# xinntao/EDVR

Measured on AMD Instinct MI355X. Metric: EDVR-L x4 5-frame 720p clips/sec, higher is better.
Workload: dtype fp32 emulated as 2xf16 (hi+lo, 22-bit operands, 4 cross products), fp32 accumulate; 1 GPU; EDVR-L x4, 5 frames, 180x320 LR -> 720x1280, batch 10/GPU, inference; clips_per_gpu=10, global_clips=10, parallelism=clip-sharded x1, no data-path collective, world_size=1, backend=single process

## Files before the change

### edvr_amd/_lib.py

```python
import ctypes
import os

_HERE = os.path.dirname(os.path.abspath(__file__))
LIB_PATH = os.environ.get('EDVR_AMD_LIB') or os.path.join(_HERE, 'lib', 'libedvr_amd.so')

c_float_p = ctypes.c_void_p
i32, i64, f32, sz = ctypes.c_int, ctypes.c_int64, ctypes.c_float, ctypes.c_size_t
vp = ctypes.c_void_p


class ConvDesc(ctypes.Structure):
    _fields_ = [
        ('x1', vp), ('x2', vp), ('c1', i32), ('c2', i32), ('x1_img_stride', i64), ('x2_img_stride', i64),
        ('x2_div', i32), ('x2_mul', i32), ('x2_add', i32), ('n', i32), ('h', i32), ('w', i32), ('wpk', vp),
        ('bias', vp), ('co', i32), ('ks', i32), ('stride', i32), ('act', i32), ('act_from', i32), ('res1', vp),
        ('res2', vp), ('res1_img_stride', i64), ('res2_img_stride', i64), ('y', vp), ('y_img_stride', i64),
        ('out_mode', i32), ('algo', i32), ('gate', vp), ('gate_img_stride', i64), ('gate_slope', f32), ('y_scale', f32),
        ('wpk_f4', vp), ('abs_sum', vp), ('abs_sum_channels', i32), ('wpk_f4s', vp), ('x_amax', vp), ('y_amax', vp),
        ('pre', vp), ('pre_img_stride', i64), ('pre_div', i32), ('pre_mul', i32), ('pre_add', i32), ('pre_n', i32),
    ]


PROTOTYPES = {
    'edvr_version': (ctypes.c_char_p, []),
# ... 9 lines not shown
    'edvr_conv2d_pack_weight_1x1s_f32': (i32, [vp, vp, i32, i32, vp]),
    'edvr_amax_f32': (i32, [vp, vp, i32, i64, i64, vp]),
    'edvr_pack_job_bytes': (sz, []),
    'edvr_conv2d_pack_weights_multi': (i32, [vp, i32, i32, i32, vp]),
    'edvr_conv2d_f32': (i32, [ctypes.POINTER(ConvDesc), vp]),
    'edvr_conv2d_gate_supported': (i32, [ctypes.POINTER(ConvDesc)]),
    'edvr_conv2d_abs_sum_supported': (i32, [ctypes.POINTER(ConvDesc)]),
    'edvr_conv2d_y_amax_supported': (i32, [ctypes.POINTER(ConvDesc)]),
    'edvr_conv2d_pre_supported': (i32, [ctypes.POINTER(ConvDesc)]),
    'edvr_conv2d_kernel_name': (i32, [ctypes.POINTER(ConvDesc), ctypes.c_char_p, sz]),
    'edvr_conv2d_executed_flops': (i32, [ctypes.POINTER(ConvDesc), ctypes.POINTER(ctypes.c_double)]),
    'edvr_dcnv2_fwd_ws_bytes': (sz, [i32] * 12),
    'edvr_dcnv2_fwd_f32': (i32, [vp] * 6 + [i32] * 12 + [i64, i64, i32, i32, vp, sz, vp]),
    'edvr_dcnv2_fwd_split_f32': (i32, [vp] * 6 + [i32] * 12 + [i64, i64, i32, i32, vp, sz, vp, vp]),
    'edvr_dcnv2_fwd_split_applies': (i32, [vp] + [i32] * 13),
    'edvr_dcnv2_fwd_kernel_name': (i32, [vp] + [i32] * 13 + [ctypes.c_char_p, sz]),
    'edvr_dcnv2_bwd_ws_bytes': (sz, [i32] * 12),
    'edvr_dcnv2_any_ws_bytes': (sz, [i32] * 13),
    'edvr_dcnv2_fwd_any': (i32, [i32] + [vp] * 6 + [i32] * 12 + [i64, i64, vp, sz, vp]),
    'edvr_dcnv2_bwd_any': (i32, [i32] + [vp] * 10 + [i32] * 12 + [i64, i64, i64, i64, vp, sz, vp]),
    'edvr_psnr_sse_f32': (i32, [vp, vp, vp, i32, i32, i32, i32, i64, i64, i32, i32, i32, vp]),
    'edvr_ssim_partials': (sz, [i32, i32, i32]),
    'edvr_ssim_f32': (i32, [vp, vp, vp, i32, i32, i32, i32, i64, i64, i32, i32, vp]),
    'edvr_frames_u8_to_f32': (i32, [vp, vp, i32, i32, i32, i32, vp, i32, vp]),
    'edvr_gather_images_f32': (i32, [vp, vp, vp, vp, i32, vp, i32, i32, vp]),
    'edvr_upsample4x_add_u8': (i32, [vp, vp, vp, i32, i32, i32, vp]),
    'edvr_f32_to_u8_hwc': (i32, [vp, vp, i32, i32, i32, i64, vp]),
    'edvr_crop_pad_frames_u8': (i32, [vp, vp, i32, i32, i32, i32, i32, i32, i32, i32, vp]),
    'edvr_crop_pad_frames_f32': (i32, [vp, vp, i32, i32, i32, i64, i32, i32, i32, i32, i32, vp]),
    'edvr_upsample4x_add_rect_f32': (i32, [vp, vp, vp, i32, i32, i32, i32, i32, i32, i32, i64, i64, i64, vp]),
# ... 89 lines not shown
```

### edvr_amd/csrc/common.h

```cpp
#pragma once
#include <hip/hip_runtime.h>

#include <cstdarg>
#include <cstdio>

#include "../../include/edvr_amd.h"

namespace edvr {

void set_error(const char *fmt, ...);

inline int check_launch(const char *what) {
  hipError_t e = hipGetLastError();
  if (e != hipSuccess) {
    set_error("%s: %s", what, hipGetErrorString(e));
    return EDVR_ERR_LAUNCH;
  }
  return EDVR_OK;
}

inline hipStream_t as_stream(edvr_stream_t s) { return reinterpret_cast<hipStream_t>(s); }

inline int cdiv(int a, int b) { return (a + b - 1) / b; }
inline int64_t cdiv64(int64_t a, int64_t b) { return (a + b - 1) / b; }
// ... 66 lines not shown
  int64_t doff_bs, dmsk_bs;
};
int dcn_fill_shape(DcnShape &s, int B, int C, int H, int W, int Co, int kh, int kw, int stride, int pad, int dil, int groups, int dg,
                   int64_t off_bs, int64_t msk_bs);

bool dcn_fused_supported(int C, int Co, int H, int W, int kh, int kw, int stride, int pad, int dil, int groups, int dg);
int dcn_fused_pack(const float *weight, float *wpk, int Co, int C, hipStream_t stream);
int dcn_fused_forward(const float *x, const float *offset, const float *mask, const float *wpk, const float *bias, float *y, int B, int C,
                      int H, int W, int Co, int dg, int64_t off_bs, int64_t msk_bs, int act, int halo, hipStream_t stream);

bool dcn_tapwin_supported(int C, int Co, int H, int W, int kh, int kw, int stride, int pad, int dil, int groups, int dg);
int dcn_tapwin_forward(const float *x, const float *offset, const float *mask, const float *wpk, const float *bias, float *y, int B, int C,
                       int H, int W, int Co, int dg, int64_t off_bs, int64_t msk_bs, int act, hipStream_t stream);

bool dcn_tapwin_split_enabled();
int dcn_tapwin_split_forward(const float *x, const float *offset, const float *mask, const float *weight, unsigned *wpk, const float *bias, float *y,
                             int B, int C, int H, int W, int Co, int dg, int64_t off_bs, int64_t msk_bs, int act, const float *xm_amax,
                             hipStream_t stream);

bool dcn_bwd_fused_supported(const DcnShape &s);
size_t dcn_bwd_fused_wbk_elems(int dg);
int dcn_bwd_fused_launch(const DcnShape &s, const float *x, const float *offset, const float *mask, const float *weight, const float *dy,
                         float *wbk, float *col, float *dx, float *doffset, float *dmask, hipStream_t stream);

__device__ inline int xcd_remap(int linear, int total) {
  const int q = total >> 3, rem = total & 7, xcd = linear & 7;
  return xcd * q + (xcd < rem ? xcd : rem) + (linear >> 3);
}
__device__ inline void xcd_block_index(int &bx, int &by, int &bz) {
  const int gx = gridDim.x, gy = gridDim.y;
  const int lin = blockIdx.x + gx * (blockIdx.y + gy * blockIdx.z);
// ... 16 lines not shown
```

### edvr_amd/csrc/dcn.hip

```cpp
#include <cstdlib>

#include "common.h"
#include "dcn_tap.h"

namespace edvr {

typedef float f32x16 __attribute__((ext_vector_type(16)));

__global__ void fill_kernel(float *__restrict__ p, float v, int64_t n) {
  for (int64_t i = (int64_t)blockIdx.x * blockDim.x + threadIdx.x; i < n; i += (int64_t)gridDim.x * blockDim.x) p[i] = v;
}

struct Merge {
  bool give01, give11;
  bool take00, take10;
};
__device__ __forceinline__ Merge merge_right(const Tap &t, bool same_plane_as_next) {
  Merge mg;
  const int lane = __lane_id();
  const int n_o00 = lane_next_i(t.o00), n_o10 = lane_next_i(t.o10);
  const int n_ok = lane_next_i((t.ok00 ? 1 : 0) | (t.ok10 ? 2 : 0));
  const bool has_next = lane < 63 && same_plane_as_next;
  mg.give01 = has_next && t.ok01 && (n_ok & 1) && n_o00 == t.o01;
  mg.give11 = has_next && t.ok11 && (n_ok & 2) && n_o10 == t.o11;
// ... 567 lines not shown
  edvr::DcnShape s;
  if (edvr::dcn_fill_shape(s, B, C, H, W, Co, kh, kw, stride, pad, dil, groups, dg, 0, 0)) return 0;
  return edvr::fwd_ws(s).total;
}

size_t edvr_dcnv2_bwd_ws_bytes(int B, int C, int H, int W, int Co, int kh, int kw, int stride, int pad, int dil, int groups,
                               int dg) {
  edvr::DcnShape s;
  if (edvr::dcn_fill_shape(s, B, C, H, W, Co, kh, kw, stride, pad, dil, groups, dg, 0, 0)) return 0;
  return edvr::bwd_ws(s).total;
}

static int dcnv2_fwd_impl(const float *x, const float *offset, const float *mask, const float *weight, const float *bias,
                          float *y, int B, int C, int H, int W, int Co, int kh, int kw, int stride, int pad, int dil, int groups,
                          int dg, int64_t offset_bstride, int64_t mask_bstride, int act, int halo_hint, void *ws, size_t ws_bytes,
                          const float *xm_amax, edvr_stream_t stream_) {
  using namespace edvr;
  EDVR_REQUIRE(x && offset && mask && weight && y, "dcnv2_fwd: null pointer");
  DcnShape s;
  int rc = dcn_fill_shape(s, B, C, H, W, Co, kh, kw, stride, pad, dil, groups, dg, offset_bstride, mask_bstride);
  if (rc) return rc;
  const FwdWs wsz = fwd_ws(s);
  if (!ws || ws_bytes < wsz.total) {
    set_error("dcnv2_fwd: workspace %zu < required %zu", ws_bytes, wsz.total);
    return EDVR_ERR_WORKSPACE;
  }
  hipStream_t stream = as_stream(stream_);
  const int K = kh * kw;
  const int64_t P = (int64_t)s.Ho * s.Wo;
  float *col = reinterpret_cast<float *>(static_cast<char *>(ws) + wsz.col);
  float *wpk = reinterpret_cast<float *>(static_cast<char *>(ws) + wsz.wpk);
  if (use_fused(s) && halo_hint == EDVR_DCN_HALO_TAPWIN && xm_amax && dcn_tapwin_split_enabled() &&
      dcn_tapwin_supported(C, Co, H, W, kh, kw, s.stride, s.pad, s.dil, groups, dg) && (reinterpret_cast<uintptr_t>(x) & 15) == 0)
    return dcn_tapwin_split_forward(x, offset, mask, weight, reinterpret_cast<unsigned *>(wpk), bias, y, B, C, H, W, Co, dg, s.off_bs, s.msk_bs, act,
                                    xm_amax, stream);
  if (use_fused(s) && halo_hint >= 0) {
    rc = dcn_fused_pack(weight, wpk, Co, C, stream);
    if (rc) return rc;
    if (halo_hint == EDVR_DCN_HALO_TAPWIN) {
      if (dcn_tapwin_supported(C, Co, H, W, kh, kw, s.stride, s.pad, s.dil, groups, dg) && (reinterpret_cast<uintptr_t>(x) & 15) == 0)
        return dcn_tapwin_forward(x, offset, mask, wpk, bias, y, B, C, H, W, Co, dg, s.off_bs, s.msk_bs, act, stream);
      halo_hint = 7;
    }
    return dcn_fused_forward(x, offset, mask, wpk, bias, y, B, C, H, W, Co, dg, s.off_bs, s.msk_bs, act, halo_hint, stream);
  }
  const int cig = C / groups, cog = Co / groups;
  const size_t wpk_g = edvr_conv2d_packed_weight_elems(cog, cig * K, 1);
  for (int g = 0; g < groups; ++g) {
    rc = edvr_conv2d_pack_weight_f32(weight + (size_t)g * cog * cig * K, wpk + g * wpk_g, cog, cig * K, 1, 0, stream_);
    if (rc) return rc;
// ... 15 lines not shown
    d.act = act;
    d.y = y + (int64_t)g * cog * P;
    d.y_img_stride = (int64_t)Co * P;
    d.out_mode = EDVR_OUT_NCHW;
    rc = conv2d_launch(d, stream);
    if (rc) return rc;
  }
  return EDVR_OK;
}

int edvr_dcnv2_fwd_f32(const float *x, const float *offset, const float *mask, const float *weight, const float *bias,
                       float *y, int B, int C, int H, int W, int Co, int kh, int kw, int stride, int pad, int dil, int groups,
                       int dg, int64_t offset_bstride, int64_t mask_bstride, int act, int halo_hint, void *ws, size_t ws_bytes,
                       edvr_stream_t stream) {
  return dcnv2_fwd_impl(x, offset, mask, weight, bias, y, B, C, H, W, Co, kh, kw, stride, pad, dil, groups, dg, offset_bstride, mask_bstride, act,
                        halo_hint, ws, ws_bytes, nullptr, stream);
}

int edvr_dcnv2_fwd_split_f32(const float *x, const float *offset, const float *mask, const float *weight, const float *bias,
                             float *y, int B, int C, int H, int W, int Co, int kh, int kw, int stride, int pad, int dil, int groups,
                             int dg, int64_t offset_bstride, int64_t mask_bstride, int act, int halo_hint, void *ws, size_t ws_bytes,
                             const float *xm_amax, edvr_stream_t stream) {
  EDVR_REQUIRE(xm_amax != nullptr, "dcnv2_fwd_split: null magnitude bound");
  return dcnv2_fwd_impl(x, offset, mask, weight, bias, y, B, C, H, W, Co, kh, kw, stride, pad, dil, groups, dg, offset_bstride, mask_bstride, act,
                        halo_hint, ws, ws_bytes, xm_amax, stream);
}

int edvr_dcnv2_fwd_split_applies(const float *x, int B, int C, int H, int W, int Co, int kh, int kw, int stride, int pad, int dil, int groups,
                                 int dg, int halo_hint) {
  using namespace edvr;
  DcnShape s;
  if (dcn_fill_shape(s, B, C, H, W, Co, kh, kw, stride, pad, dil, groups, dg, 0, 0)) return 0;
  return (use_fused(s) && halo_hint == EDVR_DCN_HALO_TAPWIN && dcn_tapwin_split_enabled() &&
          dcn_tapwin_supported(C, Co, H, W, kh, kw, s.stride, s.pad, s.dil, groups, dg) && (reinterpret_cast<uintptr_t>(x) & 15) == 0) ? 1 : 0;
}

int edvr_dcnv2_fwd_kernel_name(const float *x, int B, int C, int H, int W, int Co, int kh, int kw, int stride, int pad, int dil, int groups,
                               int dg, int halo_hint, char *buf, size_t buf_len) {
  using namespace edvr;
  EDVR_REQUIRE(buf && buf_len > 0, "dcnv2_fwd_kernel_name: null buffer");
  DcnShape s;
// ... 189 lines not shown
```

### edvr_amd/csrc/dcn_tapwin_s.hip

```cpp
#include <type_traits>

#include "common.h"
#include <cstdlib>

#include "dcn_tap.h"
#include "pack.h"

namespace edvr {

typedef float f32x16 __attribute__((ext_vector_type(16)));
typedef float f32x4 __attribute__((ext_vector_type(4)));
typedef float f32x2 __attribute__((ext_vector_type(2)));

namespace {
constexpr int TWS_TH = 8, TWS_TW = 32, TWS_RY = 2, TWS_RX = 2;
constexpr int TWS_IH = TWS_TH + 2 * TWS_RY;
constexpr int TWS_IW = (TWS_TW + 2 * TWS_RX + 3 + 3) / 4 * 4;
constexpr int TWS_PPR = TWS_IW / 4;
constexpr int TWS_HR = TWS_IH / 2;
constexpr int TWS_HB = TWS_HR * TWS_IW;
constexpr int TWS_CHS = TWS_IH * TWS_IW;
static_assert(TWS_HR * TWS_PPR <= 64 && TWS_IH == 2 * TWS_HR && TWS_CHS % 64 == 32, "window halves must fit one wave instruction");
constexpr int TWS_MAX_DG = 8;
constexpr int TWS_OOB = (int)0x80000000;
// ... 34 lines not shown

static __device__ __forceinline__ __amdgpu_buffer_rsrc_t tws_rsrc(const void *ptr, int bytes) {
  const uint64_t pv = reinterpret_cast<uint64_t>(ptr);
  const uint64_t pu = ((uint64_t)(uint32_t)__builtin_amdgcn_readfirstlane((int)(pv >> 32)) << 32) |
                      (uint32_t)__builtin_amdgcn_readfirstlane((int)(uint32_t)pv);
  return __builtin_amdgcn_make_buffer_rsrc(reinterpret_cast<void *>(pu), (short)0, bytes, TWS_RSRC_FLAGS);
}

static __device__ __forceinline__ void tws_split4(const float (&x)[4], unsigned (&o)[4]) {
  asm volatile(
      "v_fma_mixlo_f16 %0, %4, 1.0, 0\n\tv_fma_mixlo_f16 %1, %5, 1.0, 0\n\tv_fma_mixlo_f16 %2, %6, 1.0, 0\n\tv_fma_mixlo_f16 %3, %7, 1.0, 0\n\t"
      "v_fma_mixhi_f16 %0, %4, 1.0, -%0 op_sel_hi:[0,0,1]\n\tv_fma_mixhi_f16 %1, %5, 1.0, -%1 op_sel_hi:[0,0,1]\n\t"
      "v_fma_mixhi_f16 %2, %6, 1.0, -%2 op_sel_hi:[0,0,1]\n\tv_fma_mixhi_f16 %3, %7, 1.0, -%3 op_sel_hi:[0,0,1]"
      : "=&v"(o[0]), "=&v"(o[1]), "=&v"(o[2]), "=&v"(o[3])
      : "v"(x[0]), "v"(x[1]), "v"(x[2]), "v"(x[3]));
}

template <int MT, int CPG>
__global__ __launch_bounds__(256, 2) void dcn_tapwin_split_fwd_kernel(const DcnTapwinSArgs a) {
  constexpr int TH = TWS_TH, TW = TWS_TW, IH = TWS_IH, IW = TWS_IW, CHS = TWS_CHS, KK = 9, OOB = TWS_OOB;
  constexpr int MB = 32 * MT, NQ = CPG / 2, KG = CPG / 8;
  constexpr int XW = CPG * CHS;
  constexpr int WS = CPG * MB;
  constexpr int CPW = CPG / 4;
  static_assert(CPG % 4 == 0, "four waves share the channels of a group");
  __shared__ __attribute__((aligned(16))) float xw[2 * XW];
  __shared__ __attribute__((aligned(16))) unsigned wsl[2 * WS];
  __shared__ int shifts[TWS_MAX_DG * 18];
  __shared__ float tpl[4 * 3 * 64];

// ... 82 lines not shown
  };
  auto origin = [&](int g, int t, int &wy0, int &wx0) {
    const int sy = __builtin_amdgcn_readfirstlane(shifts[(g * KK + t) * 2]);
    const int sx = __builtin_amdgcn_readfirstlane(shifts[(g * KK + t) * 2 + 1]);
    const int ti = t / 3, tj = t - 3 * ti;
    wy0 = ty0 - 1 + ti + sy - TWS_RY;
    wx0 = (tx0 - 1 + tj + sx - TWS_RX) & ~3;
  };
  const i32x4 off_rsrc4 = tws_rsrc4(off_b, a.dg * 18 * P * 4), msk_rsrc4 = tws_rsrc4(msk_b, a.dg * 9 * P * 4);
  const unsigned tpl_lds = (unsigned)(size_t)(lvoid *)tpl + wave * (3 * 64 * 4);
  const int tvd = half ? tvo[1] : tvo[0];
  auto dma_taps = [&](int g, int t) {
    tws_dma4(off_rsrc4, tpl_lds, tvd, (g * 18 + 2 * t) * P * 4);
    tws_dma4(off_rsrc4, tpl_lds + 256, tvd, (g * 18 + 2 * t + 1) * P * 4);
    tws_dma4(msk_rsrc4, tpl_lds + 512, tvd, (g * 9 + t) * P * 4);
  };
  auto read_taps = [&](float (&d)[6]) {
#pragma unroll
    for (int s = 0; s < 2; ++s)
#pragma unroll
      for (int v = 0; v < 3; ++v) d[3 * s + v] = tpl[wave * 192 + v * 64 + s * 32 + j];
  };

  struct St {
    float bw[2][4];
    int addr[2];
    unsigned slow;
    unsigned slow_any;
  };
  auto state_half = [&](St &st, int s, int t, int wy0, int wx0, const float (&d)[6]) {
// ... 79 lines not shown
            v[i] = __builtin_fmaf(sw[3], gv[kg][i][3], __builtin_fmaf(sw[2], gv[kg][i][2], __builtin_fmaf(sw[1], gv[kg][i][1], sw[0] * gv[kg][i][0])));
          unsigned pk[4];
          tws_split4(v, pk);
          i32x4 bq = i32x4{(int)pk[0], (int)pk[1], (int)pk[2], (int)pk[3]};
#pragma unroll
          for (int m2 = 0; m2 < MT; ++m2)
            acc[s][m2] = __builtin_amdgcn_mfma_f32_32x32x16_f16(__builtin_bit_cast(f16x8, aw[m2]), __builtin_bit_cast(f16x8, bq), acc[s][m2], 0, 0, 0);
          asm volatile("v_alignbit_b32 %0, %0, %0, 16\n\tv_alignbit_b32 %1, %1, %1, 16\n\tv_alignbit_b32 %2, %2, %2, 16\n\tv_alignbit_b32 %3, %3, %3, 16"
                       : "+v"(bq[0]), "+v"(bq[1]), "+v"(bq[2]), "+v"(bq[3]));
#pragma unroll
          for (int m2 = 0; m2 < MT; ++m2)
            acc[s][m2] = __builtin_amdgcn_mfma_f32_32x32x16_f16(__builtin_bit_cast(f16x8, aw[m2]), __builtin_bit_cast(f16x8, bq), acc[s][m2], 0, 0, 0);
        }
      }
    } else {
      float cv[2][4][4];
      issue_cells(0, cv);
#pragma unroll
      for (int kg = 0; kg < KG; ++kg) {
        i32x4 aw[MT];
#pragma unroll
        for (int m = 0; m < MT; ++m) aw[m] = *reinterpret_cast<const i32x4 *>(wb + ((kg * 2 + half) * MB + m * 32 + j) * 4);
        i32x4 bq[2];
#pragma unroll
        for (int s = 0; s < 2; ++s) {
          const float v[4] = {sample(s, cv[s][0]), sample(s, cv[s][1]), sample(s, cv[s][2]), sample(s, cv[s][3])};
          unsigned pk[4];
          tws_split4(v, pk);
          bq[s] = i32x4{(int)pk[0], (int)pk[1], (int)pk[2], (int)pk[3]};
        }
        if (kg + 1 < KG) issue_cells(kg + 1, cv);
#pragma unroll
        for (int s = 0; s < 2; ++s)
#pragma unroll
          for (int m = 0; m < MT; ++m)
            acc[s][m] = __builtin_amdgcn_mfma_f32_32x32x16_f16(__builtin_bit_cast(f16x8, aw[m]), __builtin_bit_cast(f16x8, bq[s]), acc[s][m], 0, 0, 0);
        if (kg == 0 || KG == 1) {
          state_half(nxt, 0, tn, ny0, nx0, tnv);
#pragma unroll
          for (int i = 0; i < 4; ++i) asm volatile("" : "+v"(nxt.bw[0][i]));
          asm volatile("" : "+v"(nxt.addr[0]), "+v"(nxt.slow));
        }
        if (kg == KG - 1) {
          state_half(nxt, 1, tn, ny0, nx0, tnv);
#pragma unroll
          for (int i = 0; i < 4; ++i) asm volatile("" : "+v"(nxt.bw[1][i]));
          asm volatile("" : "+v"(nxt.addr[1]), "+v"(nxt.slow));
          state_any(nxt);
          asm volatile("" : "+s"(nxt.slow_any));
        }
#pragma unroll
        for (int s = 0; s < 2; ++s)
          asm volatile("v_alignbit_b32 %0, %0, %0, 16\n\tv_alignbit_b32 %1, %1, %1, 16\n\tv_alignbit_b32 %2, %2, %2, 16\n\tv_alignbit_b32 %3, %3, %3, 16"
                       : "+v"(bq[s][0]), "+v"(bq[s][1]), "+v"(bq[s][2]), "+v"(bq[s][3]));
#pragma unroll
        for (int s = 0; s < 2; ++s)
#pragma unroll
          for (int m = 0; m < MT; ++m)
            acc[s][m] = __builtin_amdgcn_mfma_f32_32x32x16_f16(__builtin_bit_cast(f16x8, aw[m]), __builtin_bit_cast(f16x8, bq[s]), acc[s][m], 0, 0, 0);
        __builtin_amdgcn_sched_barrier(0);
      }
    }
  };

  __syncthreads();
  const int n_steps = a.dg * KK;
  St cur, nxt;
  float tnv[6];
  int o1y, o1x;
  origin(0, 0, o1y, o1x);
  dma_x(0, 0, o1y, o1x);
  dma_w(0, 0, 0);
  dma_taps(0, 0);
  asm volatile("s_waitcnt vmcnt(0)" ::: "memory");
  read_taps(tnv);
  make_state(cur, 0, o1y, o1x, tnv);
  asm volatile("s_waitcnt lgkmcnt(0)" ::: "memory");
  int g = 0, t = 0, g1 = 0, t1 = 1;
  if (n_steps > 1) {
    origin(g1, t1, o1y, o1x);
    dma_taps(g1, t1);
    asm volatile("s_waitcnt vmcnt(0)" ::: "memory");
  }
  for (int k = 0; k < n_steps; ++k) {
    __syncthreads();
    const int g2 = (t1 == KK - 1) ? g1 + 1 : g1, t2 = (t1 == KK - 1) ? 0 : t1 + 1;
    int o2y = 0, o2x = 0;
    if (k + 1 < n_steps) {
      read_taps(tnv);
      asm volatile("s_waitcnt lgkmcnt(0)" ::: "memory");
      dma_x((k + 1) & 1, g1, o1y, o1x);
      dma_w((k + 1) & 1, g1, t1);
      if (k + 2 < n_steps) {
        origin(g2, t2, o2y, o2x);
        dma_taps(g2, t2);
      }
    }
    const float *xb = xw + (k & 1) * XW;
    const unsigned *wb = wsl + (k & 1) * WS;
    run_step(std::false_type{}, cur, xb, wb, g, t, nxt, t1, o1y, o1x, tnv);
    if (cur.slow_any) run_step(std::true_type{}, cur, xb, wb, g, t, nxt, t1, o1y, o1x, tnv);
    asm volatile("s_waitcnt vmcnt(0)" ::: "memory");
    cur = nxt;
    g = g1; t = t1; g1 = g2; t1 = t2; o1y = o2y; o1x = o2x;
  }

  const __amdgpu_buffer_rsrc_t y_rsrc = tws_rsrc(a.y + (int64_t)img * a.Co * P, a.Co * P * 4);
  const __amdgpu_buffer_rsrc_t b_rsrc = tws_rsrc(a.bias ? a.bias : a.x, a.bias ? a.Co * 4 : 0);
#pragma unroll
  for (int m = 0; m < MT; ++m) {
#pragma unroll
    for (int r4 = 0; r4 < 4; ++r4) {
// ... 58 lines not shown
  a.co_start = co_start;
  dim3 grid(a.tiles_x * a.tiles_y, co_blocks, a.B);
  if (a.C / a.dg == 16) hipLaunchKernelGGL((dcn_tapwin_split_fwd_kernel<MT, 16>), grid, dim3(256), 0, stream, a);
  else hipLaunchKernelGGL((dcn_tapwin_split_fwd_kernel<MT, 8>), grid, dim3(256), 0, stream, a);
  return check_launch("dcn_tapwin_split_fwd_kernel");
}

bool dcn_tapwin_split_enabled() {
  static const bool on = []() {
    const char *e = getenv("EDVR_DCN_SPLIT");
    return !(e && e[0] == '0');
  }();
  return on;
}

int dcn_tapwin_split_forward(const float *x, const float *offset, const float *mask, const float *weight, unsigned *wpk, const float *bias, float *y,
                             int B, int C, int H, int W, int Co, int dg, int64_t off_bs, int64_t msk_bs, int act, const float *xm_amax,
                             hipStream_t stream) {
  EDVR_REQUIRE(B <= 65535, "dcn_tapwin_split: batch %d exceeds grid.z", B);
  EDVR_REQUIRE((reinterpret_cast<uintptr_t>(x) & 15) == 0 && (reinterpret_cast<uintptr_t>(wpk) & 15) == 0, "dcn_tapwin_split: x / wpk must be 16-byte aligned");
  const int cop = (Co + 31) / 32 * 32;
  hipLaunchKernelGGL(dcn_tapwin_split_scale_kernel, dim3(1), dim3(1024), 0, stream, weight, wpk, (int64_t)Co * C * 9);
  const int64_t total = (int64_t)(C / 4) * 9 * cop;
  hipLaunchKernelGGL(dcn_tapwin_split_pack_kernel, dim3((unsigned)std::min<int64_t>(cdiv64(total, 256), 2048)), dim3(256), 0, stream, weight, wpk, Co, C, cop);
  DcnTapwinSArgs a;
  a.xm_amax = xm_amax;
  a.x = x; a.offset = offset; a.mask = mask; a.wpk = wpk; a.bias = bias; a.y = y;
  a.B = B; a.C = C; a.H = H; a.W = W; a.Co = Co; a.dg = dg; a.act = act;
  a.cop = cop;
  a.off_bs = off_bs; a.msk_bs = msk_bs;
  a.tiles_x = cdiv(W, TWS_TW);
  a.tiles_y = cdiv(H, TWS_TH);
  a.co_start = 0;
  const int full = Co / 128, rem_tiles = cdiv(Co - full * 128, 32);
  int rc = EDVR_OK;
  if (full > 0) rc = launch_tapwin_s<4>(a, 0, full, stream);
  if (rc || rem_tiles == 0) return rc;
  switch (rem_tiles) {
    case 1: return launch_tapwin_s<1>(a, full * 128, 1, stream);
// ... 8 lines not shown
```

### edvr_amd/functional.py

```python
import math
import os

import torch

from . import ops
from .ops import ACT_LRELU, ACT_NONE, ACT_RELU, ACT_SIGMOID, OUT_NCHW, OUT_PIXEL_SHUFFLE2


def _conv_geometry(m):
    ks, st = m.kernel_size, m.stride
    if (ks[0] != ks[1] or ks[0] not in (1, 3) or st[0] != st[1] or st[0] not in (1, 2) or (ks[0] == 1 and st[0] != 1)
            or tuple(m.padding) != (ks[0] // 2, ks[0] // 2) or tuple(m.dilation) != (1, 1) or m.groups != 1):
        raise NotImplementedError(
            f'edvr_amd conv kernel supports 3x3 (stride 1/2, pad 1) and 1x1 convolutions, dilation 1, groups 1; got {m}')
    return ks[0], st[0]


def _needs_grad(*ts):
    return torch.is_grad_enabled() and any(t is not None and t.requires_grad for t in ts)


def conv(m, x, *, x2=None, x2_map=None, act=ACT_NONE, act_from=0, res1=None, res2=None, out_mode=OUT_NCHW, y_scale=1.0,
         abs_sum_channels=0, ci_range=None, use_bias=True, pre=None, pre_map=None, out=None):
    ks, stride = _conv_geometry(m)
# ... 108 lines not shown


def scatter_hint_from_absmean(absmean):
    return scatter_hint_from_stats(absmean, None)


def dcn_from_packed(m, x, om, act=ACT_NONE):
    cfg = (m.stride, m.padding, m.dilation, m.groups, m.deformable_groups)
    hint = halo_hint_from_stats(getattr(m, 'last_offset_absmean', None), getattr(m, 'last_offset_rough', None), tapwin_takes(x, m))
    if _needs_grad(x, om, m.weight, m.bias):
        from . import autograd as ag
        return ag.DcnFromPackedFn.apply(x, om, m.weight, m.bias, (*cfg, act, hint, m))
    split = 2 * om.shape[1] // 3
    bias = m.bias.detach() if m.bias is not None else None
    xb = ops.input_bound(x) if (ops.F4S_INFERENCE and hint == ops.DCN_HALO_TAPWIN and tapwin_takes(x, m)) else None
    y = ops.dcnv2_forward(x, om[:, :split], om[:, split:], m.weight.detach(), bias, *cfg, act=act, halo_hint=hint, xm_bound=xb)
    if ops.F4S_INFERENCE:
        ops.linear_bound(y, m.weight, m.bias, (x,))
    return y


def upsample2x(x, scale=1.0):
    if _needs_grad(x):
        from . import autograd as ag
        return ag.Upsample2x.apply(x, scale)
    return ops.upsample2x(x, scale)


def pool_maxavg(x):
    if _needs_grad(x):
        from . import autograd as ag
# ... 31 lines not shown
```

### edvr_amd/ops.py

```python
import ctypes
import os
import weakref

import torch

from . import _lib
from ._lib import (ACT_LRELU, ACT_NONE, ACT_RELU, ACT_SIGMOID, CONV_AUTO, CONV_DIRECT, CONV_WINOGRAD, CONV_WINOGRAD_F4, CONV_WINOGRAD_F4S, OUT_NCHW,
                   OUT_PIXEL_SHUFFLE2)


def _stream():
    return ctypes.c_void_p(torch.cuda.current_stream().cuda_stream)


def _ptr(t):
    return ctypes.c_void_p(t.data_ptr()) if t is not None else ctypes.c_void_p(0)


def require_gpu(*tensors, dtypes=(torch.float32,)):
    seen = None
    for t in tensors:
        if t is None:
            continue
        if not t.is_cuda:
# ... 84 lines not shown
        _lib.check(L.edvr_conv2d_pack_weight_1x1s_f32(_ptr(w), _ptr(out), co, ci, _stream()), 'edvr_conv2d_pack_weight_1x1s_f32')
    elif f4s:
        assert k == 3, 'F(4x4,3x3) weights are for 3x3 kernels'
        out = torch.empty(L.edvr_conv2d_packed_weight_f4s_elems(co, ci), dtype=torch.int32, device=w.device)
        _lib.check(L.edvr_conv2d_pack_weight_f4s_f32(_ptr(w), _ptr(out), co, ci, 1 if transpose_flip else 0, _stream()),
                   'edvr_conv2d_pack_weight_f4s_f32')
    elif f4:
        assert k == 3, 'F(4x4,3x3) weights are for 3x3 kernels'
        out = torch.empty(L.edvr_conv2d_packed_weight_f4_elems(co, ci), dtype=torch.float32, device=w.device)
        _lib.check(L.edvr_conv2d_pack_weight_f4_f32(_ptr(w), _ptr(out), co, ci, 1 if transpose_flip else 0, _stream()),
                   'edvr_conv2d_pack_weight_f4_f32')
    else:
        out = torch.empty(L.edvr_conv2d_packed_weight_elems(co, ci, k), dtype=torch.float32, device=w.device)
        _lib.check(L.edvr_conv2d_pack_weight_f32(_ptr(w), _ptr(out), co, ci, k, 1 if transpose_flip else 0, _stream()),
                   'edvr_conv2d_pack_weight_f32')
    ent[1][key] = (ver, out, weight.data_ptr())
    return out


_PACK_CALLS = 0
_PACK_TABLES = {}


_PINNED_PACKED = set()


def pin_packed_weights(weights):
    bufs = []
    for w in weights:
        ent = _PACKED.get(id(w))
# ... 523 lines not shown
def _enc_hw(v):
    h, w = _hw(v)
    return h if h == w else (h | ((w + 1) << 16))


def _dcn_dims(x, weight, stride, pad, dil, groups, dg):
    B, C, H, W = x.shape
    Co, cig, kh, kw = weight.shape
    return [B, C, H, W, Co, kh, kw, _enc_hw(stride), _enc_hw(pad), _enc_hw(dil), groups, dg]


def _bstride(t):
    return t.stride(0) if t.shape[0] > 1 else 0


def dcnv2_forward(x, offset, mask, weight, bias, stride, pad, dil, groups, dg, act=ACT_NONE, halo_hint=0, out=None, xm_bound=None):
    dt = require_gpu(x, offset, mask, weight, bias, dtypes=tuple(DCN_DTYPES))
    L = _lib.lib()
    if not x.is_contiguous() or not weight.is_contiguous():
        raise RuntimeError('input tensor has to be contiguous')
    offset, mask = _as_planes(offset), _as_planes(mask)
    dims = _dcn_dims(x, weight, stride, pad, dil, groups, dg)
    B, C, H, W, Co, kh, kw = dims[:7]
    if C != weight.shape[1] * groups:
        raise RuntimeError(f'Input shape and kernel channels wont match: ({C} vs {weight.shape[1] * groups}).')
    (sh, sw), (ph, pw), (dh, dw) = _hw(stride), _hw(pad), _hw(dil)
    Ho = (H + 2 * ph - (dh * (kh - 1) + 1)) // sh + 1
    Wo = (W + 2 * pw - (dw * (kw - 1) + 1)) // sw + 1
    if Ho <= 0 or Wo <= 0:
        raise ValueError(f'convolution input is too small (output would be {Ho}x{Wo})')
    if tuple(offset.shape[1:]) != (dg * 2 * kh * kw, Ho, Wo):
# ... 12 lines not shown
        nbytes = L.edvr_dcnv2_any_ws_bytes(DCN_DTYPES[dt], *dims)
        ws = workspace(nbytes, x.device)
        _lib.check(L.edvr_dcnv2_fwd_any(DCN_DTYPES[dt], _ptr(x), _ptr(offset), _ptr(mask), _ptr(weight), _ptr(bias), _ptr(y), *dims,
                                        _bstride(offset), _bstride(mask), _ptr(ws), nbytes, _stream()), 'edvr_dcnv2_fwd_any')
        void_bound(y)
        return y
    nbytes = L.edvr_dcnv2_fwd_ws_bytes(*dims)
    ws = workspace(nbytes, x.device)
    name = 'dcnv2_fwd'
    split = xm_bound is not None and bool(L.edvr_dcnv2_fwd_split_applies(_ptr(x), *dims, int(halo_hint)))
    if LAUNCH_HOOK is not None:
        buf = ctypes.create_string_buffer(64)
        if L.edvr_dcnv2_fwd_kernel_name(_ptr(x), *dims, int(halo_hint), buf, 64) == 0:
            name = f'dcnv2_fwd[{"dcn_tapwin_split_fwd_kernel" if split else buf.value.decode()}]'
    common = (_ptr(x), _ptr(offset), _ptr(mask), _ptr(weight), _ptr(bias), _ptr(y), *dims, _bstride(offset), _bstride(mask), act, halo_hint, _ptr(ws), nbytes)
    if split:
        require_gpu(xm_bound)
        launch = lambda: _lib.check(L.edvr_dcnv2_fwd_split_f32(*common, _ptr(xm_bound), _stream()), 'edvr_dcnv2_fwd_split_f32')
    else:
        launch = lambda: _lib.check(L.edvr_dcnv2_fwd_f32(*common, _stream()), 'edvr_dcnv2_fwd_f32')
    _run(name, launch, 2.0 * B * Co * Ho * Wo * weight.shape[1] * kh * kw, _nb(x, offset, mask, weight, y))
    void_bound(y)
    return y


def dcnv2_backward(x, offset, mask, weight, dy, with_bias, stride, pad, dil, groups, dg, doffset=None, dmask=None,
                   scatter_hint=0, xm_bound=None, dy_bound=None):
    dt = require_gpu(x, offset, mask, weight, dy, dtypes=tuple(DCN_DTYPES))
    L = _lib.lib()
    offset, mask = _as_planes(offset), _as_planes(mask)
    dy = dy.contiguous()
# ... 855 lines not shown
```

### include/edvr_amd.h

```cpp
#ifndef EDVR_AMD_H
#define EDVR_AMD_H

#include <stddef.h>
#include <stdint.h>

#ifdef __cplusplus
extern "C" {
#endif

#define EDVR_OK 0
#define EDVR_ERR_ARG (-1)
#define EDVR_ERR_UNSUPPORTED (-2)
#define EDVR_ERR_LAUNCH (-3)
#define EDVR_ERR_WORKSPACE (-4)

typedef void *edvr_stream_t;

const char *edvr_version(void);
const char *edvr_last_error(void);
int edvr_check_device(void);

#define EDVR_ACT_NONE 0
#define EDVR_ACT_RELU 1
#define EDVR_ACT_LRELU 2
// ... 73 lines not shown
#define EDVR_HW(h, w) ((int)(h) | (((int)(w) + 1) << 16))

size_t edvr_dcnv2_fwd_ws_bytes(int B, int C, int H, int W, int Co, int kh, int kw, int stride, int pad, int dil,
                               int groups, int dg);
int edvr_dcnv2_fwd_f32(const float *x, const float *offset, const float *mask, const float *weight,
                       const float *bias, float *y, int B, int C, int H, int W, int Co, int kh, int kw, int stride,
                       int pad, int dil, int groups, int dg, int64_t offset_bstride, int64_t mask_bstride, int act,
                       int halo_hint, void *ws, size_t ws_bytes, edvr_stream_t stream);

int edvr_dcnv2_fwd_split_f32(const float *x, const float *offset, const float *mask, const float *weight, const float *bias,
                             float *y, int B, int C, int H, int W, int Co, int kh, int kw, int stride, int pad, int dil, int groups,
                             int dg, int64_t offset_bstride, int64_t mask_bstride, int act, int halo_hint, void *ws, size_t ws_bytes,
                             const float *xm_amax, edvr_stream_t stream);
int edvr_dcnv2_fwd_split_applies(const float *x, int B, int C, int H, int W, int Co, int kh, int kw, int stride, int pad, int dil, int groups,
                                 int dg, int halo_hint);
int edvr_dcnv2_fwd_kernel_name(const float *x, int B, int C, int H, int W, int Co, int kh, int kw, int stride, int pad, int dil,
                               int groups, int dg, int halo_hint, char *buf, size_t buf_len);

size_t edvr_dcnv2_bwd_ws_bytes(int B, int C, int H, int W, int Co, int kh, int kw, int stride, int pad, int dil,
                               int groups, int dg);
int edvr_dcnv2_bwd_f32(const float *x, const float *offset, const float *mask, const float *weight, const float *dy,
                       float *dx, float *doffset, float *dmask, float *dweight, float *dbias, int B, int C, int H,
                       int W, int Co, int kh, int kw, int stride, int pad, int dil, int groups, int dg,
                       int64_t offset_bstride, int64_t mask_bstride, int64_t doffset_bstride, int64_t dmask_bstride,
                       int scatter_hint, void *ws, size_t ws_bytes, edvr_stream_t stream);
int edvr_dcnv2_bwd_split_f32(const float *x, const float *offset, const float *mask, const float *weight, const float *dy,
                             float *dx, float *doffset, float *dmask, float *dweight, float *dbias, int B, int C, int H,
                             int W, int Co, int kh, int kw, int stride, int pad, int dil, int groups, int dg,
                             int64_t offset_bstride, int64_t mask_bstride, int64_t doffset_bstride, int64_t dmask_bstride,
                             int scatter_hint, void *ws, size_t ws_bytes, const float *xm_amax, const float *dy_amax,
// ... 163 lines not shown
```

Measured before the change: 99.64 clips/s.

## Cache packed DCN split weights and interleave next-step DMA between MFMAs

```diff
diff --git a/edvr_amd/_lib.py b/edvr_amd/_lib.py
--- a/edvr_amd/_lib.py
+++ b/edvr_amd/_lib.py
@@ -47,6 +47,10 @@
     'edvr_dcnv2_fwd_f32': (i32, [vp] * 6 + [i32] * 12 + [i64, i64, i32, i32, vp, sz, vp]),
     'edvr_dcnv2_fwd_split_f32': (i32, [vp] * 6 + [i32] * 12 + [i64, i64, i32, i32, vp, sz, vp, vp]),
     'edvr_dcnv2_fwd_split_applies': (i32, [vp] + [i32] * 13),
+    'edvr_dcnv2_split_packed_weight_elems': (sz, [i32, i32]),
+    'edvr_dcnv2_split_pack_weight_f32': (i32, [vp, vp, i32, i32, vp]),
+    'edvr_dcnv2_fwd_split_packed_f32': (i32, [vp] * 6 + [i32] * 12 + [i64, i64, i32, i32, vp, sz, vp, vp, vp]),
+    'edvr_dcnv2_split_pack_calls': (ctypes.c_long, []),
     'edvr_dcnv2_fwd_kernel_name': (i32, [vp] + [i32] * 13 + [ctypes.c_char_p, sz]),
     'edvr_dcnv2_bwd_ws_bytes': (sz, [i32] * 12),
     'edvr_dcnv2_any_ws_bytes': (sz, [i32] * 13),
diff --git a/edvr_amd/csrc/common.h b/edvr_amd/csrc/common.h
--- a/edvr_amd/csrc/common.h
+++ b/edvr_amd/csrc/common.h
@@ -104,7 +104,10 @@
                        int H, int W, int Co, int dg, int64_t off_bs, int64_t msk_bs, int act, hipStream_t stream);
 
 bool dcn_tapwin_split_enabled();
-int dcn_tapwin_split_forward(const float *x, const float *offset, const float *mask, const float *weight, unsigned *wpk, const float *bias, float *y,
+size_t dcn_tapwin_split_packed_elems(int Co, int C);
+int dcn_tapwin_split_pack(const float *weight, unsigned *wpk, int Co, int C, hipStream_t stream);
+long dcn_tapwin_split_pack_calls();
+int dcn_tapwin_split_forward(const float *x, const float *offset, const float *mask, const float *weight, const unsigned *wpk, const float *bias, float *y,
                              int B, int C, int H, int W, int Co, int dg, int64_t off_bs, int64_t msk_bs, int act, const float *xm_amax,
                              hipStream_t stream);
 
diff --git a/edvr_amd/csrc/dcn.hip b/edvr_amd/csrc/dcn.hip
--- a/edvr_amd/csrc/dcn.hip
+++ b/edvr_amd/csrc/dcn.hip
@@ -605,7 +605,7 @@
 static int dcnv2_fwd_impl(const float *x, const float *offset, const float *mask, const float *weight, const float *bias,
                           float *y, int B, int C, int H, int W, int Co, int kh, int kw, int stride, int pad, int dil, int groups,
                           int dg, int64_t offset_bstride, int64_t mask_bstride, int act, int halo_hint, void *ws, size_t ws_bytes,
-                          const float *xm_amax, edvr_stream_t stream_) {
+                          const float *xm_amax, const void *wpk_split, edvr_stream_t stream_) {
   using namespace edvr;
   EDVR_REQUIRE(x && offset && mask && weight && y, "dcnv2_fwd: null pointer");
   DcnShape s;
@@ -623,8 +623,9 @@
   float *wpk = reinterpret_cast<float *>(static_cast<char *>(ws) + wsz.wpk);
   if (use_fused(s) && halo_hint == EDVR_DCN_HALO_TAPWIN && xm_amax && dcn_tapwin_split_enabled() &&
       dcn_tapwin_supported(C, Co, H, W, kh, kw, s.stride, s.pad, s.dil, groups, dg) && (reinterpret_cast<uintptr_t>(x) & 15) == 0)
-    return dcn_tapwin_split_forward(x, offset, mask, weight, reinterpret_cast<unsigned *>(wpk), bias, y, B, C, H, W, Co, dg, s.off_bs, s.msk_bs, act,
-                                    xm_amax, stream);
+    return dcn_tapwin_split_forward(x, offset, mask, wpk_split ? nullptr : weight,
+                                    wpk_split ? static_cast<const unsigned *>(wpk_split) : reinterpret_cast<unsigned *>(wpk), bias, y, B, C, H, W, Co, dg,
+                                    s.off_bs, s.msk_bs, act, xm_amax, stream);
   if (use_fused(s) && halo_hint >= 0) {
     rc = dcn_fused_pack(weight, wpk, Co, C, stream);
     if (rc) return rc;
@@ -670,7 +671,7 @@
                        int dg, int64_t offset_bstride, int64_t mask_bstride, int act, int halo_hint, void *ws, size_t ws_bytes,
                        edvr_stream_t stream) {
   return dcnv2_fwd_impl(x, offset, mask, weight, bias, y, B, C, H, W, Co, kh, kw, stride, pad, dil, groups, dg, offset_bstride, mask_bstride, act,
-                        halo_hint, ws, ws_bytes, nullptr, stream);
+                        halo_hint, ws, ws_bytes, nullptr, nullptr, stream);
 }
 
 int edvr_dcnv2_fwd_split_f32(const float *x, const float *offset, const float *mask, const float *weight, const float *bias,
@@ -679,8 +680,27 @@
                              const float *xm_amax, edvr_stream_t stream) {
   EDVR_REQUIRE(xm_amax != nullptr, "dcnv2_fwd_split: null magnitude bound");
   return dcnv2_fwd_impl(x, offset, mask, weight, bias, y, B, C, H, W, Co, kh, kw, stride, pad, dil, groups, dg, offset_bstride, mask_bstride, act,
-                        halo_hint, ws, ws_bytes, xm_amax, stream);
-}
+                        halo_hint, ws, ws_bytes, xm_amax, nullptr, stream);
+}
+
+int edvr_dcnv2_fwd_split_packed_f32(const float *x, const float *offset, const float *mask, const float *weight, const float *bias,
+                                    float *y, int B, int C, int H, int W, int Co, int kh, int kw, int stride, int pad, int dil, int groups,
+                                    int dg, int64_t offset_bstride, int64_t mask_bstride, int act, int halo_hint, void *ws, size_t ws_bytes,
+                                    const float *xm_amax, const void *wpk_split, edvr_stream_t stream) {
+  EDVR_REQUIRE(xm_amax != nullptr, "dcnv2_fwd_split_packed: null magnitude bound");
+  EDVR_REQUIRE(wpk_split == nullptr || (reinterpret_cast<uintptr_t>(wpk_split) & 15) == 0, "dcnv2_fwd_split_packed: packed weights must be 16-byte aligned");
+  return dcnv2_fwd_impl(x, offset, mask, weight, bias, y, B, C, H, W, Co, kh, kw, stride, pad, dil, groups, dg, offset_bstride, mask_bstride, act,
+                        halo_hint, ws, ws_bytes, xm_amax, wpk_split, stream);
+}
+
+size_t edvr_dcnv2_split_packed_weight_elems(int Co, int C) { return edvr::dcn_tapwin_split_packed_elems(Co, C); }
+
+int edvr_dcnv2_split_pack_weight_f32(const float *weight, void *wpk, int Co, int C, edvr_stream_t stream) {
+  EDVR_REQUIRE(weight && wpk && Co > 0 && C > 0 && C % 8 == 0, "dcnv2_split_pack_weight: bad arguments");
+  return edvr::dcn_tapwin_split_pack(weight, static_cast<unsigned *>(wpk), Co, C, edvr::as_stream(stream));
+}
+
+long edvr_dcnv2_split_pack_calls(void) { return edvr::dcn_tapwin_split_pack_calls(); }
 
 int edvr_dcnv2_fwd_split_applies(const float *x, int B, int C, int H, int W, int Co, int kh, int kw, int stride, int pad, int dil, int groups,
                                  int dg, int halo_hint) {
diff --git a/edvr_amd/csrc/dcn_tapwin_s.hip b/edvr_amd/csrc/dcn_tapwin_s.hip
--- a/edvr_amd/csrc/dcn_tapwin_s.hip
+++ b/edvr_amd/csrc/dcn_tapwin_s.hip
@@ -1,6 +1,8 @@
 #include <type_traits>
+#include <utility>
 
 #include "common.h"
+#include <atomic>
 #include <cstdlib>
 
 #include "dcn_tap.h"
@@ -72,6 +74,15 @@
       "v_fma_mixhi_f16 %2, %6, 1.0, -%2 op_sel_hi:[0,0,1]\n\tv_fma_mixhi_f16 %3, %7, 1.0, -%3 op_sel_hi:[0,0,1]"
       : "=&v"(o[0]), "=&v"(o[1]), "=&v"(o[2]), "=&v"(o[3])
       : "v"(x[0]), "v"(x[1]), "v"(x[2]), "v"(x[3]));
+}
+
+template <int... I, class F>
+static __device__ __forceinline__ void tws_for_seq(std::integer_sequence<int, I...>, F &&f) {
+  (f(std::integral_constant<int, I>{}), ...);
+}
+template <int N, class F>
+static __device__ __forceinline__ void tws_for(F &&f) {
+  tws_for_seq(std::make_integer_sequence<int, N>{}, f);
 }
 
 template <int MT, int CPG>
@@ -184,6 +195,41 @@
     tws_dma4(off_rsrc4, tpl_lds, tvd, (g * 18 + 2 * t) * P * 4);
     tws_dma4(off_rsrc4, tpl_lds + 256, tvd, (g * 18 + 2 * t + 1) * P * 4);
     tws_dma4(msk_rsrc4, tpl_lds + 512, tvd, (g * 9 + t) * P * 4);
+  };
+  constexpr int ND = 2 * CPW + WNK + 3;
+  struct Req {
+    int buf, g, t, g2, t2;
+    int vo0, vo1;
+    bool more, more2;
+  } rq;
+  auto dma_piece = [&](auto PI) {
+    constexpr int p = decltype(PI)::value;
+    constexpr bool tap = p >= CPW && p < CPW + 3;
+    constexpr int i = tap ? 2 * CPW + WNK + (p - CPW) : (p < CPW ? p : p - 3);
+    if constexpr (i < 2 * CPW) {
+      constexpr int cc = i / 2, hf = i % 2;
+      if (rq.more && lane < TWS_HR * TWS_PPR) {
+        const int ch = wave * CPW + cc;
+        tws_dma16(x_rsrc4, xw_lds + (rq.buf * XW + ch * CHS + hf * TWS_HB) * 4, hf ? rq.vo1 : rq.vo0, (rq.g * CPG + ch) * P * 4);
+      }
+    } else if constexpr (i < 2 * CPW + WNK) {
+      constexpr int kk = i - 2 * CPW;
+      if (rq.more && wave + 4 * kk < WNI)
+        tws_dma16(w_rsrc4, ws_lds + (rq.buf * WS + (wave + 4 * kk) * 256) * 4, wvo[kk], 64 + ((rq.g * (CPG / 4) * KK + rq.t) * a.cop + co_blk) * 16);
+    } else {
+      constexpr int v = i - 2 * CPW - WNK;
+      if (rq.more2) {
+        if constexpr (v == 0) asm volatile("s_waitcnt lgkmcnt(0)" ::: "memory");
+        tws_dma4(v < 2 ? off_rsrc4 : msk_rsrc4, tpl_lds + 256 * v, tvd, (v < 2 ? rq.g2 * 18 + 2 * rq.t2 + v : rq.g2 * 9 + rq.t2) * P * 4);
+      }
+    }
+  };
+  auto request = [&](int buf, int g, int t, int wy0, int wx0, int g2, int t2, bool more, bool more2) {
+    const int sh = (wy0 * a.W + wx0) * 4;
+    const bool colok = (unsigned)(wx0 + d_c) < (unsigned)a.W;
+    rq.vo0 = (colok && (unsigned)(wy0 + d_r) < (unsigned)a.H) ? rel0 + sh : OOB;
+    rq.vo1 = (colok && (unsigned)(wy0 + d_r + TWS_HR) < (unsigned)a.H) ? rel0 + sh + TWS_HR * a.W * 4 : OOB;
+    rq.buf = buf; rq.g = g; rq.t = t; rq.g2 = g2; rq.t2 = t2; rq.more = more; rq.more2 = more2;
   };
   auto read_taps = [&](float (&d)[6]) {
 #pragma unroll
@@ -293,10 +339,20 @@
         }
       }
     } else {
+      constexpr int NS = (KG * 4 - 3) * MT;
+      auto spread = [&](auto NI) {
+        constexpr int n = decltype(NI)::value;
+        constexpr int lo = n < NS ? n * ND / NS : ND, hi = n < NS ? (n + 1) * ND / NS : ND;
+        if constexpr (hi > lo) {
+          __builtin_amdgcn_sched_barrier(0);
+          tws_for<hi - lo>([&](auto PI) { dma_piece(std::integral_constant<int, lo + decltype(PI)::value>{}); });
+          __builtin_amdgcn_sched_barrier(0);
+        }
+      };
       float cv[2][4][4];
       issue_cells(0, cv);
-#pragma unroll
-      for (int kg = 0; kg < KG; ++kg) {
+      tws_for<KG>([&](auto KGI) {
+        constexpr int kg = decltype(KGI)::value;
         i32x4 aw[MT];
 #pragma unroll
         for (int m = 0; m < MT; ++m) aw[m] = *reinterpret_cast<const i32x4 *>(wb + ((kg * 2 + half) * MB + m * 32 + j) * 4);
@@ -308,12 +364,12 @@
           tws_split4(v, pk);
           bq[s] = i32x4{(int)pk[0], (int)pk[1], (int)pk[2], (int)pk[3]};
         }
-        if (kg + 1 < KG) issue_cells(kg + 1, cv);
-#pragma unroll
-        for (int s = 0; s < 2; ++s)
-#pragma unroll
-          for (int m = 0; m < MT; ++m)
-            acc[s][m] = __builtin_amdgcn_mfma_f32_32x32x16_f16(__builtin_bit_cast(f16x8, aw[m]), __builtin_bit_cast(f16x8, bq[s]), acc[s][m], 0, 0, 0);
+        if constexpr (kg + 1 < KG) issue_cells(kg + 1, cv);
+        tws_for<2 * MT>([&](auto NI) {
+          constexpr int s = decltype(NI)::value / MT, m = decltype(NI)::value % MT;
+          acc[s][m] = __builtin_amdgcn_mfma_f32_32x32x16_f16(__builtin_bit_cast(f16x8, aw[m]), __builtin_bit_cast(f16x8, bq[s]), acc[s][m], 0, 0, 0);
+          spread(std::integral_constant<int, kg * 4 * MT + decltype(NI)::value>{});
+        });
         if (kg == 0 || KG == 1) {
           state_half(nxt, 0, tn, ny0, nx0, tnv);
 #pragma unroll
@@ -332,13 +388,13 @@
         for (int s = 0; s < 2; ++s)
           asm volatile("v_alignbit_b32 %0, %0, %0, 16\n\tv_alignbit_b32 %1, %1, %1, 16\n\tv_alignbit_b32 %2, %2, %2, 16\n\tv_alignbit_b32 %3, %3, %3, 16"
                        : "+v"(bq[s][0]), "+v"(bq[s][1]), "+v"(bq[s][2]), "+v"(bq[s][3]));
-#pragma unroll
-        for (int s = 0; s < 2; ++s)
-#pragma unroll
-          for (int m = 0; m < MT; ++m)
-            acc[s][m] = __builtin_amdgcn_mfma_f32_32x32x16_f16(__builtin_bit_cast(f16x8, aw[m]), __builtin_bit_cast(f16x8, bq[s]), acc[s][m], 0, 0, 0);
+        tws_for<2 * MT>([&](auto NI) {
+          constexpr int s = decltype(NI)::value / MT, m = decltype(NI)::value % MT;
+          acc[s][m] = __builtin_amdgcn_mfma_f32_32x32x16_f16(__builtin_bit_cast(f16x8, aw[m]), __builtin_bit_cast(f16x8, bq[s]), acc[s][m], 0, 0, 0);
+          spread(std::integral_constant<int, (kg * 4 + 2) * MT + decltype(NI)::value>{});
+        });
         __builtin_amdgcn_sched_barrier(0);
-      }
+      });
     }
   };
 
@@ -365,16 +421,9 @@
     __syncthreads();
     const int g2 = (t1 == KK - 1) ? g1 + 1 : g1, t2 = (t1 == KK - 1) ? 0 : t1 + 1;
     int o2y = 0, o2x = 0;
-    if (k + 1 < n_steps) {
-      read_taps(tnv);
-      asm volatile("s_waitcnt lgkmcnt(0)" ::: "memory");
-      dma_x((k + 1) & 1, g1, o1y, o1x);
-      dma_w((k + 1) & 1, g1, t1);
-      if (k + 2 < n_steps) {
-        origin(g2, t2, o2y, o2x);
-        dma_taps(g2, t2);
-      }
-    }
+    if (k + 1 < n_steps) read_taps(tnv);
+    if (k + 2 < n_steps) origin(g2, t2, o2y, o2x);
+    request((k + 1) & 1, g1, t1, o1y, o1x, g2, t2, k + 1 < n_steps, k + 2 < n_steps);
     const float *xb = xw + (k & 1) * XW;
     const unsigned *wb = wsl + (k & 1) * WS;
     run_step(std::false_type{}, cur, xb, wb, g, t, nxt, t1, o1y, o1x, tnv);
@@ -463,15 +512,31 @@
   return on;
 }
 
-int dcn_tapwin_split_forward(const float *x, const float *offset, const float *mask, const float *weight, unsigned *wpk, const float *bias, float *y,
+size_t dcn_tapwin_split_packed_elems(int Co, int C) { return 16 + (size_t)C * 9 * ((Co + 31) / 32 * 32); }
+
+static std::atomic<long> tws_pack_calls{0};
+long dcn_tapwin_split_pack_calls() { return tws_pack_calls.load(); }
+
+int dcn_tapwin_split_pack(const float *weight, unsigned *wpk, int Co, int C, hipStream_t stream) {
+  EDVR_REQUIRE((reinterpret_cast<uintptr_t>(wpk) & 15) == 0, "dcn_tapwin_split_pack: wpk must be 16-byte aligned");
+  const int cop = (Co + 31) / 32 * 32;
+  tws_pack_calls.fetch_add(1);
+  hipLaunchKernelGGL(dcn_tapwin_split_scale_kernel, dim3(1), dim3(1024), 0, stream, weight, wpk, (int64_t)Co * C * 9);
+  const int64_t total = (int64_t)(C / 4) * 9 * cop;
+  hipLaunchKernelGGL(dcn_tapwin_split_pack_kernel, dim3((unsigned)std::min<int64_t>(cdiv64(total, 256), 2048)), dim3(256), 0, stream, weight, wpk, Co, C, cop);
+  return check_launch("dcn_tapwin_split_pack_kernel");
+}
+
+int dcn_tapwin_split_forward(const float *x, const float *offset, const float *mask, const float *weight, const unsigned *wpk, const float *bias, float *y,
                              int B, int C, int H, int W, int Co, int dg, int64_t off_bs, int64_t msk_bs, int act, const float *xm_amax,
                              hipStream_t stream) {
   EDVR_REQUIRE(B <= 65535, "dcn_tapwin_split: batch %d exceeds grid.z", B);
   EDVR_REQUIRE((reinterpret_cast<uintptr_t>(x) & 15) == 0 && (reinterpret_cast<uintptr_t>(wpk) & 15) == 0, "dcn_tapwin_split: x / wpk must be 16-byte aligned");
   const int cop = (Co + 31) / 32 * 32;
-  hipLaunchKernelGGL(dcn_tapwin_split_scale_kernel, dim3(1), dim3(1024), 0, stream, weight, wpk, (int64_t)Co * C * 9);
-  const int64_t total = (int64_t)(C / 4) * 9 * cop;
-  hipLaunchKernelGGL(dcn_tapwin_split_pack_kernel, dim3((unsigned)std::min<int64_t>(cdiv64(total, 256), 2048)), dim3(256), 0, stream, weight, wpk, Co, C, cop);
+  if (weight) {
+    const int rcp = dcn_tapwin_split_pack(weight, const_cast<unsigned *>(wpk), Co, C, stream);
+    if (rcp) return rcp;
+  }
   DcnTapwinSArgs a;
   a.xm_amax = xm_amax;
   a.x = x; a.offset = offset; a.mask = mask; a.wpk = wpk; a.bias = bias; a.y = y;
diff --git a/edvr_amd/functional.py b/edvr_amd/functional.py
--- a/edvr_amd/functional.py
+++ b/edvr_amd/functional.py
@@ -146,7 +146,7 @@
     split = 2 * om.shape[1] // 3
     bias = m.bias.detach() if m.bias is not None else None
     xb = ops.input_bound(x) if (ops.F4S_INFERENCE and hint == ops.DCN_HALO_TAPWIN and tapwin_takes(x, m)) else None
-    y = ops.dcnv2_forward(x, om[:, :split], om[:, split:], m.weight.detach(), bias, *cfg, act=act, halo_hint=hint, xm_bound=xb)
+    y = ops.dcnv2_forward(x, om[:, :split], om[:, split:], m.weight.detach(), bias, *cfg, act=act, halo_hint=hint, xm_bound=xb, packed_from=m.weight)
     if ops.F4S_INFERENCE:
         ops.linear_bound(y, m.weight, m.bias, (x,))
     return y
diff --git a/edvr_amd/ops.py b/edvr_amd/ops.py
--- a/edvr_amd/ops.py
+++ b/edvr_amd/ops.py
@@ -122,6 +122,34 @@
         out = torch.empty(L.edvr_conv2d_packed_weight_elems(co, ci, k), dtype=torch.float32, device=w.device)
         _lib.check(L.edvr_conv2d_pack_weight_f32(_ptr(w), _ptr(out), co, ci, k, 1 if transpose_flip else 0, _stream()),
                    'edvr_conv2d_pack_weight_f32')
+    ent[1][key] = (ver, out, weight.data_ptr())
+    return out
+
+
+def pack_dcn_split_weight(weight):
+    require_gpu(weight)
+    key, wid, ver = ('dcn_split',), id(weight), weight._version
+    ent = _PACKED.get(wid)
+    if ent is not None and ent[0]() is weight:
+        hit = ent[1].get(key)
+        if hit is not None and hit[0] == ver and hit[2] == weight.data_ptr():
+            return hit[1]
+    else:
+        ent = (weakref.ref(weight, lambda _r, wid=wid: _PACKED.pop(wid, None)), {})
+        _PACKED[wid] = ent
+    L = _lib.lib()
+    w = weight.detach()
+    if not w.is_contiguous():
+        w = w.contiguous()
+    co, ci, k, k2 = w.shape
+    assert k == 3 and k2 == 3 and ci % 8 == 0, 'the split tap-window kernel takes 3x3 weights over whole 8-channel groups'
+    n_el = L.edvr_dcnv2_split_packed_weight_elems(co, ci)
+    stale = ent[1].get(key)
+    if stale is not None and stale[1].numel() == n_el and stale[1].device == w.device and _sole_owner(stale):
+        out = stale[1]
+    else:
+        out = torch.empty(n_el, dtype=torch.int32, device=w.device)
+    _lib.check(L.edvr_dcnv2_split_pack_weight_f32(_ptr(w), _ptr(out), co, ci, _stream()), 'edvr_dcnv2_split_pack_weight_f32')
     ent[1][key] = (ver, out, weight.data_ptr())
     return out
 
@@ -675,7 +703,8 @@
     return t.stride(0) if t.shape[0] > 1 else 0
 
 
-def dcnv2_forward(x, offset, mask, weight, bias, stride, pad, dil, groups, dg, act=ACT_NONE, halo_hint=0, out=None, xm_bound=None):
+def dcnv2_forward(x, offset, mask, weight, bias, stride, pad, dil, groups, dg, act=ACT_NONE, halo_hint=0, out=None, xm_bound=None,
+                  wpk_split=None, packed_from=None):
     dt = require_gpu(x, offset, mask, weight, bias, dtypes=tuple(DCN_DTYPES))
     L = _lib.lib()
     if not x.is_contiguous() or not weight.is_contiguous():
@@ -718,7 +747,17 @@
         if L.edvr_dcnv2_fwd_kernel_name(_ptr(x), *dims, int(halo_hint), buf, 64) == 0:
             name = f'dcnv2_fwd[{"dcn_tapwin_split_fwd_kernel" if split else buf.value.decode()}]'
     common = (_ptr(x), _ptr(offset), _ptr(mask), _ptr(weight), _ptr(bias), _ptr(y), *dims, _bstride(offset), _bstride(mask), act, halo_hint, _ptr(ws), nbytes)
-    if split:
+    if split and wpk_split is None and packed_from is not None:
+        wpk_split = pack_dcn_split_weight(packed_from)
+    if split and wpk_split is not None:
+        require_gpu(xm_bound)
+        require_gpu(wpk_split, dtypes=(torch.int32,))
+        if wpk_split.numel() != L.edvr_dcnv2_split_packed_weight_elems(Co, C):
+            raise RuntimeError(f'wpk_split holds {wpk_split.numel()} elements, the packing of a ({Co}, {C}, 3, 3) weight has '
+                               f'{L.edvr_dcnv2_split_packed_weight_elems(Co, C)}')
+        launch = lambda: _lib.check(L.edvr_dcnv2_fwd_split_packed_f32(*common, _ptr(xm_bound), _ptr(wpk_split), _stream()),
+                                    'edvr_dcnv2_fwd_split_packed_f32')
+    elif split:
         require_gpu(xm_bound)
         launch = lambda: _lib.check(L.edvr_dcnv2_fwd_split_f32(*common, _ptr(xm_bound), _stream()), 'edvr_dcnv2_fwd_split_f32')
     else:
diff --git a/include/edvr_amd.h b/include/edvr_amd.h
--- a/include/edvr_amd.h
+++ b/include/edvr_amd.h
@@ -111,6 +111,13 @@
                              const float *xm_amax, edvr_stream_t stream);
 int edvr_dcnv2_fwd_split_applies(const float *x, int B, int C, int H, int W, int Co, int kh, int kw, int stride, int pad, int dil, int groups,
                                  int dg, int halo_hint);
+size_t edvr_dcnv2_split_packed_weight_elems(int Co, int C);
+int edvr_dcnv2_split_pack_weight_f32(const float *weight, void *wpk, int Co, int C, edvr_stream_t stream);
+int edvr_dcnv2_fwd_split_packed_f32(const float *x, const float *offset, const float *mask, const float *weight, const float *bias,
+                                    float *y, int B, int C, int H, int W, int Co, int kh, int kw, int stride, int pad, int dil, int groups,
+                                    int dg, int64_t offset_bstride, int64_t mask_bstride, int act, int halo_hint, void *ws, size_t ws_bytes,
+                                    const float *xm_amax, const void *wpk_split, edvr_stream_t stream);
+long edvr_dcnv2_split_pack_calls(void);
 int edvr_dcnv2_fwd_kernel_name(const float *x, int B, int C, int H, int W, int Co, int kh, int kw, int stride, int pad, int dil,
                                int groups, int dg, int halo_hint, char *buf, size_t buf_len);
 
```

Result: no change. 99.50 clips/s, median of 5 (-0.1%).
